# gerbenvoshol/fqzcomp5

Measured on AMD Instinct MI355X. Metric: input MB/s encode+decode, 100MB blocks, -3 and -5; bit-exact vs CPU, higher is better.
Workload: dtype u8

## Files before the change

### fqzcomp5_amd/csrc/block.cpp

```cpp
#include <atomic>
#include <cstdio>
#include <algorithm>
#include <cstdlib>
#include <cstring>
#include <exception>
#include <functional>
#include <thread>
#include <deque>
#include <memory>
#include <vector>

#include "../../include/fqz5_block.h"
#include "rans_codec.hpp"
#include "fqz_codec.hpp"
#include "seq_codec.hpp"
#include "seq_cm.h"
#include "lzp_codec.hpp"
#include "names.hpp"
#include "host_dec.hpp"
#include "rans_format.hpp"

namespace fqz5 {

GpuCtx &gpu();
// ... 22 lines not shown

SeqEncReq seq_req(const fqz5_section &S, int m) {
    static const int slevel[] = {10, 12, 12, 13, 14}, both[] = {0, 0, 1, 1, 1};
    SeqEncReq r;
    r.d_in = S.in;
    r.n = S.in_size;
    r.lens = S.rec_len;
    r.nrec = S.nrec;
    r.k = slevel[m - SEQ10];
    r.both = both[m - SEQ10];
    return r;
}
int seq_strat(int m) {
    static const int slevel[] = {10, 12, 12, 13, 14}, both[] = {0, 0, 1, 1, 1};
    return (slevel[m - SEQ10] << 4) | (both[m - SEQ10] << 3) | 1;
}

int method_order(int m, uint32_t fixed_len) {
    static const int ord[] = {0, 1, 64, 65, 128, 129, 192, 193};
    if (m >= RANS0 && m <= RANS193) return ord[m - RANS0];
    return int((fixed_len << 8) + 9);
}

uint32_t metrics_method(fqz5_trial_state &st, int sec, uint32_t avail) {
    fqz5_section_stats &s = st.sec[sec];
    if (s.review <= 0) {
        s.review = FQZ5_METRICS_REVIEW;
        s.trial = FQZ5_METRICS_TRIAL;
        std::memset(s.usize, 0, sizeof s.usize);
        std::memset(s.csize, 0, sizeof s.csize);
        std::memset(s.count, 0, sizeof s.count);
    }
    if (s.trial > 0) return avail;
    if (s.trial > -99999) {
        int best_m = 0;
        double best = 1e30;
        for (int m = 0; m < FQZ5_M_LAST; m++) {
            if (s.usize[m] && best > (s.csize[m] + 1.0) / s.usize[m]) {
                best = (s.csize[m] + 1.0) / s.usize[m];
                best_m = m;
            }
        }
        s.method_used = best_m;
        s.trial = -99999;
        return 1u << best_m;
    }
    s.review--;
    return 1u << s.method_used;
}

}

struct TrySession {
    std::vector<CompressReq> reqs;
    std::vector<std::vector<int>> req_of;
    std::vector<FqzEncReq> fqz;
    std::vector<uint64_t> fqz_lb;
    std::vector<std::vector<int>> fqz_of;
    std::vector<SeqEncReq> seq;
    std::vector<uint64_t> seq_lb;
    std::vector<uint64_t> fqz_ub, seq_ub;
    std::vector<char> fqz_skip, seq_skip;
    std::vector<std::vector<int>> seq_of;
    std::vector<uint32_t> upper;
    std::deque<std::vector<uint32_t>> recs;
    std::vector<NameEnc> names;
    std::vector<std::vector<int>> name_of;
    bool open = false;
    bool aux = false;
};

FqzEncReq fqz_req(const fqz5_section &S, int m, std::deque<std::vector<uint32_t>> &keep) {
    FqzEncReq r;
    r.d_in = S.in;
    r.n = S.in_size;
    r.nrec = S.nrec;
    keep.emplace_back(S.rec_len, S.rec_len + std::max(S.nrec, 0));
    r.lens = keep.back().data();
    if (S.rec_flags)
        keep.emplace_back(S.rec_flags, S.rec_flags + std::max(S.nrec, 0));
    else
        keep.emplace_back(size_t(std::max(S.nrec, 0)), 0u);
    r.flags = keep.back().data();
    r.d_seq = S.seq;
    r.vers = 4;
    r.strat = m - FQZ0;
    return r;
}
thread_local TrySession t_sess;

void encode_name_jobs(GpuCtx &g, const fqz5_section *secs, const std::vector<int> &which,
                      const std::vector<int> &meth, std::vector<NameEnc> &out) {
// ... 17 lines not shown
        g.download(hb, S.in, S.in_size);
        hipEvent_t e;
        FQZ5_HIP(hipEventCreateWithFlags(&e, hipEventDisableTiming));
        evs.push_back(e);
        FQZ5_HIP(hipEventRecord(e, g.stream));
        host.push_back(hb);
    }
    std::vector<const uint8_t *> h(which.size()), d(which.size());
    std::vector<uint32_t> lens(which.size());
    std::vector<hipEvent_t> ready(which.size());
    for (size_t k = 0; k < which.size(); k++) {
        h[k] = host[size_t(host_of[k])];
        ready[k] = evs[size_t(host_of[k])];
        d[k] = secs[which[k]].in;
        lens[k] = secs[which[k]].in_size;
    }
    names_encode_batch(g, out, h, d, lens, meth, &ready);
    g.sync();
}

std::atomic<int> g_prune{0};
std::atomic<int> g_bounds{0};
std::atomic<uint64_t> g_fqz_tried{0}, g_fqz_pruned{0};
std::atomic<uint64_t> g_chains_host{0}, g_chains_gpu{0};

template <class LB>
std::vector<char> prune_plan(const std::vector<CompressReq> &reqs,
                             const std::vector<std::vector<int>> &of, int mlo, int mhi,
                             size_t nreq, LB lb) {
    std::vector<char> skip(nreq, 0);
    const int nsec = int(of.size());
    std::vector<int> F;
    for (int i = 0; i < nsec; i++)
        for (int m = mlo; m <= mhi; m++)
            if (of[i][m] >= 0) { F.push_back(i); break; }
    if (F.size() != size_t(FQZ5_METRICS_TRIAL)) return skip;
    auto rsize = [&](int i, int m) -> int64_t {
        const int ri = t_sess.req_of[i][m];
        return ri >= 0 && reqs[size_t(ri)].ok ? int64_t(layout_size(reqs[size_t(ri)].out)) : -1;
    };
    std::vector<int64_t> best(F.size(), -1);
    for (size_t k = 0; k < F.size(); k++)
        for (int m = 1; m < mlo; m++) {
            const int64_t z = rsize(F[k], m);
            if (z >= 0 && (best[k] < 0 || z < best[k])) best[k] = z;
        }
// ... 81 lines not shown
    out2[0] = g_chains_host.load();
    out2[1] = g_chains_gpu.load();
}

void fqz5_rans_chain_counts(uint64_t *out2) { rans_chain_counts(out2); }
void fqz5_rans_enc_chain_counts(uint64_t *out2) { rans_enc_chain_counts(out2); }

void fqz5_rans_variant_counts(uint64_t *dec, uint64_t *dec_hedged, uint64_t *enc, int *ndec,
                              int *nenc) {
    rans_variant_counts(dec, dec_hedged, enc, ndec, nenc);
}
const char *fqz5_rans_variant_name(int dir, int i) { return rans_variant_name(dir, i); }

int fqz5_seq_path_counts(uint64_t *out, int n) { return seq_path_counts(out, n); }

void fqz5_trial_counts(uint64_t *out2) {
    out2[0] = g_fqz_tried.load();
    out2[1] = g_fqz_pruned.load();
}

void fqz5_trial_schedule(const int32_t *sec_ids, int nsec, const uint32_t *avail,
                         const fqz5_trial_state *st, uint32_t *masks_out) {
    fqz5_trial_state s = *st;
    for (int i = 0; i < nsec; i++) {
        fqz5_section_stats &ss = s.sec[sec_ids[i]];
        if (ss.review <= 0) {
            ss.review = FQZ5_METRICS_REVIEW;
            ss.trial = FQZ5_METRICS_TRIAL;
        }
        masks_out[i] = 0;
        if (ss.trial > 0) {
            masks_out[i] = avail[sec_ids[i]];
            ss.trial--;
        } else if (ss.trial > -99999) {
            ss.trial = -99999;
        } else {
            ss.review--;
        }
    }
}

using host::now_ms;
using host::now_ns;
using host::step_trace;

int fqz5_sections_try(const fqz5_section *secs, int nsec, const uint32_t *masks,
                      uint32_t *sizes) {
    const double t0 = step_trace() ? now_ms() : 0;
    try {
        GpuCtx &g = gpu();
        if (t_sess.open) {
            g.reset();
            gpu_aux_reset_all();
        }
        t_sess = TrySession();
        for (int i = 0; i < nsec; i++) {
            if (masks[i] & ~(RANS_MASK | FQZ_MASK | SEQ_MASK | NAME_MASK | (1u << LZP3)))
                throw GpuError("fqz5_sections_try: method mask has SEQ_CUSTOM (not in this build)");
            if ((masks[i] & NAME_MASK) && secs[i].sec != FQZ5_SEC_NAME)
                throw GpuError("fqz5_sections_try: name methods need a name section");
            if (secs[i].sec == FQZ5_SEC_NAME && (masks[i] & ~NAME_MASK))
                throw GpuError("fqz5_sections_try: a name section takes name methods only");
            if ((masks[i] & SEQ_MASK) && (secs[i].sec != FQZ5_SEC_SEQ || !secs[i].rec_len))
                throw GpuError("fqz5_sections_try: SEQ methods need a sequence section with records");
            if ((masks[i] & FQZ_MASK) && (secs[i].sec != FQZ5_SEC_QUAL || !secs[i].rec_len))
                throw GpuError("fqz5_sections_try: FQZ methods need a quality section with records");
        }
        std::vector<CompressReq> &reqs = t_sess.reqs;
        t_sess.req_of.assign(nsec, std::vector<int>(FQZ5_M_LAST, -1));
        t_sess.fqz_of.assign(nsec, std::vector<int>(FQZ5_M_LAST, -1));
        t_sess.seq_of.assign(nsec, std::vector<int>(FQZ5_M_LAST, -1));
        t_sess.name_of.assign(nsec, std::vector<int>(FQZ5_M_LAST, -1));
        std::vector<int> name_sec, name_meth;
        std::vector<int> lzp_sec;
        std::vector<CompressReq> sreq;
        std::vector<int> sreq_sec;
        for (int i = 0; i < nsec; i++) {
            const fqz5_section &S = secs[i];
// ... 23 lines not shown
                CompressReq r;
                r.d_in = S.in;
                r.n = S.in_size;
                r.order = method_order(m, S.fixed_len);
                r.cap = compress_bound(r.n, r.order);
                if (m == RANSXN1) {
                    sreq_sec.push_back(i);
                    sreq.push_back(std::move(r));
                    continue;
                }
                t_sess.req_of[i][m] = int(reqs.size());
                reqs.push_back(std::move(r));
            }
        }
        static const bool no_aux = std::getenv("FQZ5_NO_AUX") != nullptr;
        std::vector<FqzEncReq> &fq = t_sess.fqz;
        std::vector<SeqEncReq> &sq = t_sess.seq;
        auto join_stripes = [&] {
            for (size_t k = 0; k < sreq.size(); k++) {
                t_sess.req_of[size_t(sreq_sec[k])][RANSXN1] = int(reqs.size());
                reqs.push_back(std::move(sreq[k]));
            }
            sreq.clear();
        };
        if ((!fq.empty() || !sq.empty() || !lzp_sec.empty() || !sreq.empty() || !name_sec.empty()) &&
            !no_aux) {
            t_sess.aux = true;
            GpuCtx &ga = gpu_aux(0), &gb = gpu_aux(2), &gc = gpu_aux(1);
            size_t nsq = std::min<size_t>(sq.size(), size_t(AUX_NSEQ));
            {
                uint64_t mx = 1;
                for (const SeqEncReq &q : sq) mx = std::max<uint64_t>(mx, q.n);
                size_t fr = 0, tot = 0;
                if (hipMemGetInfo(&fr, &tot) != hipSuccess || !tot) tot = size_t(64) << 30;
                const uint64_t fit = (uint64_t(tot) / 4) / (120 * mx);
                nsq = std::max<size_t>(1, std::min<size_t>(nsq, size_t(fit)));
            }
            std::vector<std::vector<SeqEncReq>> sqg(nsq);
            for (size_t k = 0; k < sq.size(); k++) sqg[k % std::max<size_t>(nsq, 1)].push_back(sq[k]);
            std::vector<CompressReq> lzr;
            std::vector<std::vector<int>> lzr_of(size_t(nsec), std::vector<int>(FQZ5_M_LAST, -1));
            std::vector<std::exception_ptr> err(2 + nsq);
            auto on = [t0](GpuCtx &c, std::exception_ptr &e, auto &&fn) {
                return std::thread([&c, &e, fn, t0] {
                    try {
                        FQZ5_HIP(hipSetDevice(c.device));
// ... 31 lines not shown
            std::vector<CompressReq> plain, rest;
            for (size_t k = 0; k < reqs.size(); k++)
                if ((reqs[k].order & ~1) == 0 && reqs[k].n >= (1u << 20)) plain_at.push_back(k);
            if (plain_at.size() == reqs.size()) plain_at.clear();
            for (size_t k : plain_at) is_plain[k] = 1;
            if (!plain_at.empty())
                for (size_t k = 0; k < reqs.size(); k++)
                    (is_plain[k] ? plain : rest).push_back(std::move(reqs[k]));
            GpuCtx &gp = gpu_aux(AUX_PLAIN);
            gp.prof.on = g.prof.on;
            std::exception_ptr perr;
            std::thread tp = on(gp, perr, [&] { if (!plain.empty()) compress_batch(gp, plain); });
            double tc = 0, tpl = 0;
            try {
                compress_batch(g, plain_at.empty() ? reqs : rest);
                if (!plain_at.empty()) {
                    size_t q = 0;
                    for (size_t k = 0; k < reqs.size(); k++)
                        if (!is_plain[k]) reqs[k] = std::move(rest[q++]);
                }
                tc = step_trace() ? now_ms() : 0;
                tp.join();
                tpl = step_trace() ? now_ms() : 0;
            } catch (...) {
                if (tp.joinable()) tp.join();
                for (auto &t : th) t.join();
                ts.join();
                tn.join();
                throw;
            }
            if (perr) {
                for (auto &t : th) t.join();
                ts.join();
                tn.join();
                std::rethrow_exception(perr);
            }
            for (size_t q = 0; q < plain_at.size(); q++) reqs[plain_at[q]] = std::move(plain[q]);
            g.prof.enc_ms += gp.prof.enc_ms;
            g.prof.enc_launches += gp.prof.enc_launches;
            g.prof.enc_bytes += gp.prof.enc_bytes;
            gp.prof = KernelProfile();
            if (step_trace() && !plain_at.empty())
                std::fprintf(stderr, "sections_try: %zu plain rANS candidates on a helper, "
                             "done %.1f ms after the others\n", plain_at.size(), tpl - tc);
            tc = std::max(tc, tpl);
            for (auto &t : th) t.join();
            ts.join();
            tn.join();
            if (serr) std::rethrow_exception(serr);
            if (nerr) std::rethrow_exception(nerr);
            join_stripes();
            if (step_trace())
                std::fprintf(stderr, "sections_try: rANS candidates %.1f ms, helpers waited "
                             "%.1f ms more\n", tc - t0, now_ms() - tc);
            for (auto &e : err)
                if (e) std::rethrow_exception(e);
            for (size_t k = 0; k < sq.size(); k++)
                sq[k] = std::move(sqg[k % std::max<size_t>(nsq, 1)][k / std::max<size_t>(nsq, 1)]);
            for (int i : lzp_sec) {
                t_sess.req_of[size_t(i)][LZP3] = int(reqs.size());
                reqs.push_back(std::move(lzr[size_t(lzr_of[size_t(i)][LZP3])]));
            }
            std::vector<char> skip_f(fq.size(), 0), skip_s(sq.size(), 0);
            if (g_bounds.load()) {
                for (size_t k = 0; k < fq.size(); k++) skip_f[k] = fqz_size_lower_bound(fq[k]) > 0;
                for (size_t k = 0; k < sq.size(); k++) skip_s[k] = seq_size_upper_bound(sq[k]) > 0;
            } else if (g_prune.load()) {
                skip_f = prune_plan(reqs, t_sess.fqz_of, FQZ0, FQZ4, fq.size(),
                                    [&](size_t k) { return fqz_size_lower_bound(fq[k]); });
                skip_s = prune_plan(reqs, t_sess.seq_of, SEQ10, SEQ14B, sq.size(),
                                    [&](size_t k) { return seq_size_lower_bound(sq[k]); });
            }
            std::exception_ptr ferr;
            std::thread tf = on(ga, ferr, [&] { if (!fq.empty()) fqz_encode_finish(ga, fq, &skip_f); });
// ... 3 lines not shown
            } catch (...) {
                tf.join();
                throw;
            }
            tf.join();
            if (ferr) std::rethrow_exception(ferr);
            t_sess.fqz_skip.insert(t_sess.fqz_skip.end(), skip_f.begin(), skip_f.end());
            t_sess.seq_skip.insert(t_sess.seq_skip.end(), skip_s.begin(), skip_s.end());
            for (size_t k = 0; k < fq.size(); k++) {
                t_sess.fqz_lb.push_back(skip_f[k] ? fqz_size_lower_bound(fq[k]) : 0);
                t_sess.fqz_ub.push_back(skip_f[k] ? fqz_size_upper_bound(fq[k]) : 0);
            }
            for (size_t k = 0; k < sq.size(); k++) {
                t_sess.seq_lb.push_back(skip_s[k] ? seq_size_lower_bound(sq[k]) : 0);
                t_sess.seq_ub.push_back(skip_s[k] ? seq_size_upper_bound(sq[k]) : 0);
            }
            g_fqz_tried += fq.size() + sq.size();
            for (char c : skip_f) g_fqz_pruned += c ? 1 : 0;
            for (char c : skip_s) g_fqz_pruned += c ? 1 : 0;
        } else {
            join_stripes();
            add_lzp3(g, secs, lzp_sec, reqs, t_sess.req_of);
            compress_batch(g, reqs);
            encode_name_jobs(g, secs, name_sec, name_meth, t_sess.names);
            if (!fq.empty()) fqz_encode_batch(g, fq);
            if (!sq.empty()) seq_encode_batch(g, sq);
            t_sess.fqz_lb.assign(fq.size(), 0);
            t_sess.seq_lb.assign(sq.size(), 0);
            t_sess.fqz_ub.assign(fq.size(), 0);
            t_sess.seq_ub.assign(sq.size(), 0);
            t_sess.fqz_skip.assign(fq.size(), 0);
            t_sess.seq_skip.assign(sq.size(), 0);
            g_fqz_tried += fq.size() + sq.size();
        }
        t_sess.open = true;
        if (step_trace())
            std::fprintf(stderr, "sections_try: %.1f ms (device / pinned allocations so far %llu, "
                         "frees %llu)\n", now_ms() - t0,
                         (unsigned long long)ChunkPool::alloc_calls().load(),
                         (unsigned long long)ChunkPool::free_calls().load());
        t_sess.upper.assign(size_t(nsec) * FQZ5_M_LAST, 0);
        for (int i = 0; i < nsec; i++) {
            uint32_t stale = UINT32_MAX;
            for (int m = 0; m < FQZ5_M_LAST; m++) {
                const int ri = t_sess.req_of[i][m], fi = t_sess.fqz_of[i][m];
                const int si = t_sess.seq_of[i][m], ni = t_sess.name_of[i][m];
// ... 12 lines not shown
                }
                if (fi >= 0) {
                    const uint64_t lb = t_sess.fqz_lb[size_t(fi)];
                    sz = t_sess.fqz[size_t(fi)].ok ? layout_size(t_sess.fqz[size_t(fi)].out)
                         : lb ? uint32_t(std::min<uint64_t>(lb, UINT32_MAX - 1)) : 0;
                }
                uint32_t up = sz;
                if (si >= 0 && !t_sess.seq[size_t(si)].ok && t_sess.seq_ub[size_t(si)])
                    up = uint32_t(std::min<uint64_t>(t_sess.seq_ub[size_t(si)], UINT32_MAX - 1));
                if (fi >= 0 && !t_sess.fqz[size_t(fi)].ok && t_sess.fqz_ub[size_t(fi)])
                    up = uint32_t(std::min<uint64_t>(t_sess.fqz_ub[size_t(fi)], UINT32_MAX - 1));
                sizes[size_t(i) * FQZ5_M_LAST + m] = sz;
                t_sess.upper[size_t(i) * FQZ5_M_LAST + m] = up;
            }
        }
        return 0;
    } catch (const std::exception &e) {
        fqz5_set_error(e.what());
        t_sess = TrySession();
        try { gpu().reset(); } catch (...) {}
        try { gpu_aux_reset_all(); } catch (...) {}
        return -1;
    }
}

void fqz5_trial_replay(const int32_t *sec_ids, const uint32_t *in_sizes,
                       const uint32_t *sizes, int nsec, const uint32_t *avail,
                       fqz5_trial_state *st, int32_t *methods_out,
                       uint32_t *tried_out) {
    for (int i = 0; i < nsec; i++) {
        const int sec = sec_ids[i];
        fqz5_section_stats &ss = st->sec[sec];
        const uint32_t methods = metrics_method(*st, sec, avail[sec]);
        const bool in_trial = ss.trial > 0;
        uint32_t best_sz = UINT32_MAX;
        int best_m = 0;
        for (int m = 0; m < FQZ5_M_LAST; m++) {
            if (!(methods & (1u << m))) continue;
            const uint32_t out_len = sizes[size_t(i) * FQZ5_M_LAST + m];
            if (best_sz > out_len) { best_sz = out_len; best_m = m; }
        }
        if (!in_trial && __builtin_popcount(methods) == 1) best_m = __builtin_ctz(methods);
        if (in_trial) {
            for (int m = 0; m < FQZ5_M_LAST; m++) {
                if (!(methods & (1u << m)) || ss.trial <= 0) continue;
                ss.usize[m] += in_sizes[i];
// ... 9 lines not shown

int fqz5_sections_commit(const fqz5_section *secs, int nsec, const int32_t *methods,
                         fqz5_section_result *res) {
    const double t0 = step_trace() ? now_ms() : 0;
    try {
        GpuCtx &g = gpu();
        if (!t_sess.open || int(t_sess.req_of.size()) != nsec)
            throw GpuError("fqz5_sections_commit: no matching fqz5_sections_try");
        std::vector<CompressReq> late;
        std::vector<int> late_of(nsec, -1), late_fqz_of(nsec, -1), late_seq_of(nsec, -1);
        std::vector<FqzEncReq> late_fqz;
        std::vector<SeqEncReq> late_seq;
        std::vector<int> late_lzp;
        std::vector<std::vector<int>> late_lzp_of(nsec, std::vector<int>(FQZ5_M_LAST, -1));
        std::vector<int> late_name_sec, late_name_meth, late_name_of(nsec, -1);
        auto coded_fqz = [&](int i, int m) {
            const int f = t_sess.fqz_of[i][m];
            return f >= 0 && !(size_t(f) < t_sess.fqz_skip.size() && t_sess.fqz_skip[size_t(f)]);
        };
        auto coded_seq = [&](int i, int m) {
            const int q = t_sess.seq_of[i][m];
            return q >= 0 && !(size_t(q) < t_sess.seq_skip.size() && t_sess.seq_skip[size_t(q)]);
        };
        for (int i = 0; i < nsec; i++) {
            const int m = methods[i];
            if (m <= 0 || m >= FQZ5_M_LAST || t_sess.req_of[i][m] >= 0 || coded_fqz(i, m) ||
                coded_seq(i, m) || t_sess.name_of[i][m] >= 0)
                continue;
            if (is_name_method(m) && secs[i].sec == FQZ5_SEC_NAME) {
                late_name_of[i] = int(late_name_sec.size());
                late_name_sec.push_back(i);
                late_name_meth.push_back(m);
                continue;
            }
            if (is_seqcm(m) && secs[i].sec == FQZ5_SEC_SEQ && secs[i].rec_len) {
                late_seq_of[i] = int(late_seq.size());
                late_seq.push_back(seq_req(secs[i], m));
                continue;
            }
            if (is_fqz(m) && secs[i].sec == FQZ5_SEC_QUAL && secs[i].rec_len) {
                late_fqz_of[i] = int(late_fqz.size());
                late_fqz.push_back(fqz_req(secs[i], m, t_sess.recs));
                continue;
            }
            if (m == LZP3 && secs[i].sec == FQZ5_SEC_SEQ) {
                late_lzp.push_back(i);
// ... 115 lines not shown
        std::thread([old = std::make_unique<TrySession>(std::move(t_sess))]() mutable {
            old.reset();
        }).detach();
        t_sess = TrySession();
        if (step_trace())
            std::fprintf(stderr, "sections_commit: late encodes %.1f ms, write %.1f ms, sync "
                         "%.1f ms, release %.1f ms\n", t1 - t0, t2 - t1, t3 - t2, now_ms() - t3);
        return 0;
    } catch (const std::exception &e) {
        fqz5_set_error(e.what());
        t_sess = TrySession();
        try { gpu().reset(); } catch (...) {}
        return -1;
    }
}

int fqz5_encode_sections(const fqz5_section *secs, int nsec, const uint32_t *avail,
                         fqz5_trial_state *st, fqz5_section_result *res) {
    std::vector<uint32_t> sizes(size_t(nsec) * FQZ5_M_LAST), masks(nsec);
    std::vector<int32_t> ids(nsec), meth(nsec);
    std::vector<uint32_t> ins(nsec);
    for (int i = 0; i < nsec; i++) { ids[i] = secs[i].sec; ins[i] = secs[i].in_size; }
    for (int i = 0; i < nsec; i++) masks[i] = avail[secs[i].sec];
    if (fqz5_sections_try(secs, nsec, masks.data(), sizes.data())) return -1;
    fqz5_trial_replay(ids.data(), ins.data(), sizes.data(), nsec, avail, st, meth.data(),
                      nullptr);
    return fqz5_sections_commit(secs, nsec, meth.data(), res);
}

int fqz5_decode_sections(const fqz5_section *secs, int nsec, fqz5_section_result *res) {
    struct ExitTrace {
        double t;
        ~ExitTrace() {
            if (t) std::fprintf(stderr, "decode_sections: entry to exit %.1f ms\n", now_ms() - t);
        }
    } exit_trace{step_trace() ? now_ms() : 0.0};
    try {
        GpuCtx &g = gpu();
        const bool trace = step_trace();
        const double t0 = now_ms();
        size_t tot = 0;
        for (int i = 0; i < nsec; i++) tot += secs[i].in_size;
        uint8_t *host = g.staging.alloc(tot + 1);
        size_t off = 0;
        for (int i = 0; i < nsec; i++) {
            g.download(host + off, secs[i].in, secs[i].in_size);
            off += secs[i].in_size;
// ... 395 lines not shown
```

### fqzcomp5_amd/sections.py

```python
from __future__ import annotations

import ctypes as C

import numpy as np

from . import lib as _lib

M_LAST = 31
SEC_NAME, SEC_SEQ, SEC_QUAL = 0, 2, 3
RANS0, RANS1, RANS64, RANS65, RANS128, RANS129, RANS192, RANS193, RANSXN1 = range(1, 10)
LZP3 = 10
TLZP3 = 11
TOK3_3, TOK3_5, TOK3_7, TOK3_9 = range(12, 16)
TOK3_3_LZP, TOK3_5_LZP, TOK3_7_LZP, TOK3_9_LZP = range(16, 20)
NAME_MASK = sum(1 << m for m in range(TLZP3, TOK3_9_LZP + 1))
SEQ10, SEQ12, SEQ12B, SEQ13B, SEQ14B = range(20, 25)
FQZ0, FQZ1, FQZ2, FQZ3, FQZ4 = range(26, 31)
RANS_MASK = sum(1 << m for m in range(RANS0, RANSXN1 + 1))
FQZ_MASK = sum(1 << m for m in range(FQZ0, FQZ4 + 1))
SEQ_MASK = sum(1 << m for m in range(SEQ10, SEQ14B + 1))
WORK_MASK = FQZ_MASK | SEQ_MASK | (1 << LZP3)

PRESET_MASKS = {
    1: {SEC_NAME: [TLZP3],
# ... 69 lines not shown


def _load():
    global _bound
    so = _lib.load()
    if not _bound:
        so.fqz5_trial_init.argtypes = [C.POINTER(TrialState)]
        so.fqz5_set_trial_prune.restype = C.c_int
        so.fqz5_set_trial_prune.argtypes = [C.c_int]
        so.fqz5_set_trial_bounds.restype = C.c_int
        so.fqz5_set_trial_bounds.argtypes = [C.c_int]
        so.fqz5_arenas_release.restype = C.c_int
        so.fqz5_arenas_release.argtypes = []
        so.fqz5_sections_try_upper.restype = C.c_int
        so.fqz5_sections_try_upper.argtypes = [C.POINTER(C.c_uint32), C.c_int]
        so.fqz5_trial_counts.argtypes = [C.POINTER(C.c_uint64)]
        so.fqz5_trial_schedule.argtypes = [C.POINTER(C.c_int32), C.c_int,
                                           C.POINTER(C.c_uint32), C.POINTER(TrialState),
                                           C.POINTER(C.c_uint32)]
        so.fqz5_sections_try.argtypes = [C.POINTER(Section), C.c_int,
                                         C.POINTER(C.c_uint32),
                                         C.POINTER(C.c_uint32)]
        so.fqz5_sections_try.restype = C.c_int
        so.fqz5_trial_replay.argtypes = [C.POINTER(C.c_int32), C.POINTER(C.c_uint32),
                                         C.POINTER(C.c_uint32), C.c_int,
                                         C.POINTER(C.c_uint32), C.POINTER(TrialState),
                                         C.POINTER(C.c_int32), C.POINTER(C.c_uint32)]
        so.fqz5_sections_commit.argtypes = [C.POINTER(Section), C.c_int,
                                            C.POINTER(C.c_int32),
                                            C.POINTER(SectionResult)]
        so.fqz5_sections_commit.restype = C.c_int
        so.fqz5_decode_sections.argtypes = [C.POINTER(Section), C.c_int,
                                            C.POINTER(SectionResult)]
        so.fqz5_decode_sections.restype = C.c_int
        _bound = True
    return so


def masks(level: int, seq_cm: bool = False, full: bool = False) -> np.ndarray:
    av = np.zeros(4, np.uint32)
    for sec, ms in PRESET_MASKS[level].items():
        for m in ms:
            if m not in BUILT or (m in SEQ_PARAMS and not (seq_cm or full)):
                continue
            av[sec] |= np.uint32(1 << m)
    return av


def new_state() -> TrialState:
    st = TrialState()
    _load().fqz5_trial_init(C.byref(st))
    return st


def _arr(t, xs):
    return (t * len(xs))(*xs)


def trial_schedule(sec_ids, avail: np.ndarray, state: TrialState) -> np.ndarray:
    so = _load()
    ids = np.ascontiguousarray(sec_ids, np.int32)
    av = np.ascontiguousarray(avail, np.uint32)
    out = np.zeros(len(ids), np.uint32)
    so.fqz5_trial_schedule(ids.ctypes.data_as(C.POINTER(C.c_int32)), len(ids),
                           av.ctypes.data_as(C.POINTER(C.c_uint32)), C.byref(state),
                           out.ctypes.data_as(C.POINTER(C.c_uint32)))
    return out


def sections_try(secs: list[Section], masks: np.ndarray) -> np.ndarray:
    so = _load()
    sizes = np.zeros(len(secs) * M_LAST, np.uint32)
    av = np.ascontiguousarray(masks, np.uint32)
    assert len(av) == len(secs)
    _lib.after_torch()
    rc = so.fqz5_sections_try(_arr(Section, secs), len(secs),
                              av.ctypes.data_as(C.POINTER(C.c_uint32)),
                              sizes.ctypes.data_as(C.POINTER(C.c_uint32)))
    if rc:
        raise _lib.NativeError("fqz5_sections_try: " + _lib.last_error())
    return sizes.reshape(len(secs), M_LAST)


def trial_replay(sec_ids, in_sizes, sizes: np.ndarray, avail: np.ndarray,
                 state: TrialState, tried: np.ndarray | None = None) -> np.ndarray:
    so = _load()
    n = len(sec_ids)
    ids = np.ascontiguousarray(sec_ids, np.int32)
    ins = np.ascontiguousarray(in_sizes, np.uint32)
    sz = np.ascontiguousarray(sizes, np.uint32).reshape(-1)
    av = np.ascontiguousarray(avail, np.uint32)
    out = np.zeros(n, np.int32)
    so.fqz5_trial_replay(ids.ctypes.data_as(C.POINTER(C.c_int32)),
                         ins.ctypes.data_as(C.POINTER(C.c_uint32)),
                         sz.ctypes.data_as(C.POINTER(C.c_uint32)), n,
                         av.ctypes.data_as(C.POINTER(C.c_uint32)),
                         C.byref(state), out.ctypes.data_as(C.POINTER(C.c_int32)),
                         None if tried is None else
                         tried.ctypes.data_as(C.POINTER(C.c_uint32)))
    return out


def sections_try_bounds(secs: list[Section], masks: np.ndarray):
    so = _load()
    prev = so.fqz5_set_trial_bounds(1)
    try:
        lo = sections_try(secs, masks)
    finally:
        so.fqz5_set_trial_bounds(prev)
    hi = np.zeros(len(secs) * M_LAST, np.uint32)
    if so.fqz5_sections_try_upper(hi.ctypes.data_as(C.POINTER(C.c_uint32)), len(secs)):
        raise _lib.NativeError("fqz5_sections_try_upper: " + _lib.last_error())
    return lo, hi.reshape(len(secs), M_LAST)


def _first_min_open(lo, hi, ratios: bool = False) -> list:
    w = min(range(len(lo)), key=lambda j: (lo[j], j))
    out = []
    for j in range(len(lo)):
        if j == w or (lo[j] == hi[j] and lo[w] == hi[w]):
            continue
        gap = hi[w] * (1 + 1e-9) if ratios else hi[w]
        if (j < w and not gap < lo[j]) or (j > w and not gap <= lo[j]):
            out.append(j)
    return out + [w] if out else []


def _first_min_fixed(lo, hi, ratios: bool = False) -> bool:
    return not _first_min_open(lo, hi, ratios)

# ... 192 lines not shown
    if group is None:
        group = dist.group.WORLD
    ws, rk = _world(group)
    if ws == 1:
        return local, in_sizes, sec_ids, 0
    pack = np.zeros((local.shape[0], M_LAST + 2), np.int64)
    pack[:, :M_LAST] = local
    pack[:, M_LAST] = in_sizes
    pack[:, M_LAST + 1] = sec_ids
    rows = xchg(pack, group)
    allp = np.concatenate(rows, 0)
    off = sum(int(r.shape[0]) for r in rows[:rk])
    return (allp[:, :M_LAST].astype(np.uint32), allp[:, M_LAST].astype(np.uint32),
            allp[:, M_LAST + 1].astype(np.int32), off)


def encode_run(secs: list[Section], avail: np.ndarray, state: TrialState,
               group=None, speculate: bool = True, prune: bool = True,
               bounds: bool = False):
    ins = np.array([s.in_size for s in secs], np.uint32)
    ids = np.array([s.sec for s in secs], np.int32)
    av = np.asarray(avail, np.uint32)
    SPEC = RANS_MASK | NAME_MASK
    if speculate and not (av & WORK_MASK).any():
        masks = av[ids]
        prune = False
    else:
        blank = np.zeros((len(secs), M_LAST), np.uint32)
        _, _, g_ids0, off = exchange_sizes(blank, ins, ids, group)
        sched_all = trial_schedule(g_ids0, avail, state)
        sched = sched_all[off:off + len(secs)]
        NAME_WORK = 1 << TLZP3
        masks = ((av[ids] & np.uint32(SPEC & ~NAME_WORK & 0xFFFFFFFF)) |
                 (sched & np.uint32(WORK_MASK | NAME_WORK)) if speculate else sched)
        for fam in (FQZ_MASK, SEQ_MASK):
            rows = np.nonzero(sched_all & fam)[0]
            if len(rows) == 0:
                continue
            prune = prune and speculate and len(rows) == TRIAL_WINDOW and \
                bool(((rows >= off) & (rows < off + len(secs))).all())
        if bounds and _world(group)[0] == 1 and (sched_all & WORK_MASK).any() and \
                bounds_usable(g_ids0, sched_all, state, final=True):
            global last_bounds_decided
            state0 = _copy_state(state)
            lo, hi = sections_try_bounds(secs, masks)
            tried = np.zeros(len(secs), np.uint32)
            meth_all = trial_replay(ids, ins, lo, avail, state, tried)
            last_bounds_decided = trial_decided(lo, hi, ids, ins, tried, sched_all, state0,
                                                final=True)
            if last_bounds_decided:
                return sections_commit(secs, meth_all), meth_all, lo, tried, 0
            C.memmove(C.byref(state), C.byref(state0), C.sizeof(TrialState))
    so = _load()
    prev = so.fqz5_set_trial_prune(1 if prune else 0)
    try:
        local = sections_try(secs, masks)
    finally:
        so.fqz5_set_trial_prune(prev)
    g_sizes, g_ins, g_ids, off = exchange_sizes(local, ins, ids, group)
    tried = np.zeros(len(g_ids), np.uint32)
    meth_all = trial_replay(g_ids, g_ins, g_sizes, avail, state, tried)
    meth = meth_all[off:off + len(secs)]
    res = sections_commit(secs, meth)
    return res, meth_all, g_sizes, tried, off


def _chunks(rows, sizes, budget: int):
    out, cur, tot = [], [], 0
    for i in rows:
        if cur and tot + int(sizes[i]) > budget:
            out.append(cur)
            cur, tot = [], 0
        cur.append(i)
        tot += int(sizes[i])
    if cur:
        out.append(cur)
    return out


# ... 58 lines not shown
            tried = np.zeros(len(g_ids), np.uint32)
            meth_all = trial_replay(g_ids, g_ins, g_sizes, avail, state, tried)
        global last_bounds_decided
        last_bounds_decided = ok
        if not ok:
            print(f"[sections] size intervals do not decide the trial ({why[0] if why else ''}): "
                  "trying again with exact sizes", file=sys.stderr, flush=True)
            C.memmove(C.byref(state), C.byref(state0), C.sizeof(TrialState))
            lo, _ = try_all(False)
            g_sizes, g_ins, g_ids, off = exchange_sizes(lo, ins, ids, group)
            tried = np.zeros(len(g_ids), np.uint32)
            meth_all = trial_replay(g_ids, g_ins, g_sizes, avail, state, tried)
    meth = meth_all[off:off + len(secs)]
    if bounds and last_bounds_decided and session:
        return sections_commit(secs, meth), meth_all, g_sizes, tried, off
    if so.fqz5_arenas_release():
        raise _lib.NativeError("fqz5_arenas_release: " + _lib.last_error())
    res = []
    for ch in _chunks(range(len(secs)), ins, max(commit_bytes, chunk_bytes)):
        part = [secs[i] for i in ch]
        sections_try(part, np.zeros(len(ch), np.uint32))
        res += sections_commit(part, meth[ch])
    return res, meth_all, g_sizes, tried, off


def _world(group):
    import torch.distributed as dist
    if group is None or not dist.is_available() or not dist.is_initialized():
        return 1, 0
    return dist.get_world_size(group), dist.get_rank(group)


def allreduce_min(a: np.ndarray, group) -> np.ndarray:
    if _world(group)[0] == 1:
        return a
    parts = xchg(np.ascontiguousarray(a, np.int64), group)
    return np.minimum.reduce(parts).astype(a.dtype)


def work_share(methods: list[int], world: int, rank: int) -> int:
    m = 0
    for j, meth in enumerate(sorted(methods)):
        if j % world == rank:
            m |= 1 << meth
    return m

# ... 454 lines not shown
```

### include/fqz5_block.h

```cpp
#ifndef FQZ5_BLOCK_H
#define FQZ5_BLOCK_H
#include <stdint.h>

#ifdef __cplusplus
extern "C" {
#endif

#define FQZ5_M_LAST 31
#define FQZ5_SEC_NAME 0
#define FQZ5_SEC_LEN 1
#define FQZ5_SEC_SEQ 2
#define FQZ5_SEC_QUAL 3
#define FQZ5_SEC_LAST 4
#define FQZ5_METRICS_REVIEW 100
#define FQZ5_METRICS_TRIAL 3

typedef struct {
    uint64_t usize[FQZ5_M_LAST], csize[FQZ5_M_LAST];
    int32_t review, trial;
    int32_t count[FQZ5_M_LAST];
    int32_t method_used;
} fqz5_section_stats;

typedef struct {
// ... 17 lines not shown
    int32_t method;
    int32_t strat;
    int32_t status;
    uint32_t clen;
    uint32_t usize;
} fqz5_section_result;

void fqz5_trial_init(fqz5_trial_state *st);

int fqz5_encode_sections(const fqz5_section *secs, int n, const uint32_t *avail,
                         fqz5_trial_state *st, fqz5_section_result *res);

void fqz5_trial_schedule(const int32_t *sec_ids, int n, const uint32_t *avail,
                         const fqz5_trial_state *st, uint32_t *masks_out);
int fqz5_sections_try(const fqz5_section *secs, int n, const uint32_t *masks,
                      uint32_t *sizes);
void fqz5_trial_replay(const int32_t *sec_ids, const uint32_t *in_sizes,
                       const uint32_t *sizes, int n, const uint32_t *avail,
                       fqz5_trial_state *st, int32_t *methods_out,
                       uint32_t *tried_out );
int fqz5_sections_commit(const fqz5_section *secs, int n, const int32_t *methods,
                         fqz5_section_result *res);

int fqz5_set_trial_prune(int on);
int fqz5_set_trial_bounds(int on);
int fqz5_sections_try_upper(uint32_t *upper, int nsec);
int fqz5_arenas_release(void);
void fqz5_trial_counts(uint64_t *out2);

int fqz5_decode_sections(const fqz5_section *secs, int n, fqz5_section_result *res);


#define FQZ5_FREAD2 128

void fqz5_name_flags(const char *names, uint32_t name_len, int nrec, uint32_t *flags);

int fqz5_block_lengths(const uint32_t *len, int nrec, int32_t fixed_len, uint8_t *out,
                       uint32_t cap);

typedef struct {
    int32_t nrec;
    const uint8_t *name;
    uint32_t name_size;
    const uint8_t *lengths;
    uint32_t lengths_size;
    const uint8_t *seq;
// ... 38 lines not shown
```

Before: 3562.

## Stage trial encoding so follower sections only encode the predicted winner

Adds a staged trial path. Sections still inside the trial window are encoded with every candidate method. Sections whose method is already settled are restricted to that method, and sections that follow a trial window get no encodes in the first pass. After the trial-window encodes finish, the best rANS method is picked from the accumulated stats and only that method is encoded for the followers, split across a helper context. This cuts redundant candidate encodes per batch, at the cost of a second encode stage and possible mispredictions that must be fixed up in replay.

Result: faster. 4326, median of 6 (+21.5%).

```diff
diff --git a/fqzcomp5_amd/csrc/block.cpp b/fqzcomp5_amd/csrc/block.cpp
--- a/fqzcomp5_amd/csrc/block.cpp
+++ b/fqzcomp5_amd/csrc/block.cpp
@@ -68,6 +68,19 @@
     return int((fixed_len << 8) + 9);
 }
 
+int pick_method(const fqz5_section_stats &s, uint32_t among) {
+    int best_m = 0;
+    double best = 1e30;
+    for (int m = 0; m < FQZ5_M_LAST; m++) {
+        if (!(among & (1u << m))) continue;
+        if (s.usize[m] && best > (s.csize[m] + 1.0) / s.usize[m]) {
+            best = (s.csize[m] + 1.0) / s.usize[m];
+            best_m = m;
+        }
+    }
+    return best_m;
+}
+
 uint32_t metrics_method(fqz5_trial_state &st, int sec, uint32_t avail) {
     fqz5_section_stats &s = st.sec[sec];
     if (s.review <= 0) {
@@ -79,20 +92,98 @@
     }
     if (s.trial > 0) return avail;
     if (s.trial > -99999) {
-        int best_m = 0;
-        double best = 1e30;
-        for (int m = 0; m < FQZ5_M_LAST; m++) {
-            if (s.usize[m] && best > (s.csize[m] + 1.0) / s.usize[m]) {
-                best = (s.csize[m] + 1.0) / s.usize[m];
-                best_m = m;
-            }
-        }
-        s.method_used = best_m;
+        s.method_used = pick_method(s, ~0u);
         s.trial = -99999;
-        return 1u << best_m;
+        return 1u << s.method_used;
     }
     s.review--;
     return 1u << s.method_used;
+}
+
+enum TrialStep { STEP_TRIAL, STEP_DECIDE, STEP_KEEP };
+TrialStep trial_step(fqz5_section_stats &ss, bool *fresh = nullptr) {
+    if (ss.review <= 0) {
+        ss.review = FQZ5_METRICS_REVIEW;
+        ss.trial = FQZ5_METRICS_TRIAL;
+        if (fresh) *fresh = true;
+    }
+    if (ss.trial > 0) {
+        ss.trial--;
+        return STEP_TRIAL;
+    }
+    if (ss.trial > -99999) {
+        ss.trial = -99999;
+        return STEP_DECIDE;
+    }
+    ss.review--;
+    return STEP_KEEP;
+}
+
+struct Decision {
+    int kind = 0;
+    bool fresh = false;
+    std::vector<int> rows;
+    std::vector<int> follow;
+};
+
+void staged_walk(const int32_t *sec_ids, int nsec, const uint32_t *avail,
+                 const fqz5_trial_state *st, int32_t *roles, uint32_t *masks, int32_t *window,
+                 std::vector<Decision> *decs) {
+    fqz5_trial_state s = *st;
+    int cur[FQZ5_SEC_LAST], nwin[FQZ5_SEC_LAST], settled[FQZ5_SEC_LAST];
+    bool open[FQZ5_SEC_LAST];
+    for (int k = 0; k < FQZ5_SEC_LAST; k++) {
+        cur[k] = -1;
+        nwin[k] = 0;
+        settled[k] = s.sec[k].method_used;
+        open[k] = false;
+    }
+    std::vector<Decision> local;
+    std::vector<Decision> &D = decs ? *decs : local;
+    for (int i = 0; i < nsec; i++) {
+        const int k = sec_ids[i];
+        fqz5_section_stats &ss = s.sec[k];
+        const bool staged = k == FQZ5_SEC_SEQ || k == FQZ5_SEC_QUAL;
+        bool fresh = false;
+        const TrialStep step = trial_step(ss, &fresh);
+        window[i] = -1;
+        if (step == STEP_TRIAL) {
+            roles[i] = staged ? FQZ5_ROLE_TRIAL : FQZ5_ROLE_OTHER;
+            masks[i] = avail[k];
+            if (!staged) continue;
+            if (!open[k]) {
+                Decision d;
+                d.kind = k;
+                d.fresh = fresh;
+                cur[k] = int(D.size());
+                D.push_back(d);
+                open[k] = true;
+                nwin[k]++;
+            }
+            D[size_t(cur[k])].rows.push_back(i);
+            window[i] = nwin[k] - 1;
+            continue;
+        }
+        if (!staged) {
+            roles[i] = FQZ5_ROLE_OTHER;
+            masks[i] = 0;
+            continue;
+        }
+        if (step == STEP_DECIDE && !open[k]) {
+            settled[k] = pick_method(st->sec[k], ~0u);
+            cur[k] = -1;
+        }
+        open[k] = false;
+        if (cur[k] >= 0) {
+            roles[i] = FQZ5_ROLE_FOLLOW;
+            masks[i] = 0;
+            window[i] = nwin[k] - 1;
+            D[size_t(cur[k])].follow.push_back(i);
+        } else {
+            roles[i] = FQZ5_ROLE_SETTLED;
+            masks[i] = 1u << settled[k];
+        }
+    }
 }
 
 }
@@ -114,6 +205,7 @@
     std::vector<std::vector<int>> name_of;
     bool open = false;
     bool aux = false;
+    std::vector<int> predicted;
 };
 
 FqzEncReq fqz_req(const fqz5_section &S, int m, std::deque<std::vector<uint32_t>> &keep) {
@@ -177,6 +269,19 @@
 std::atomic<int> g_prune{0};
 std::atomic<int> g_bounds{0};
 std::atomic<uint64_t> g_fqz_tried{0}, g_fqz_pruned{0};
+std::atomic<int> g_staged{-1};
+std::atomic<uint64_t> g_staged_n[4];
+std::atomic<uint64_t> g_staged_dec[FQZ5_SEC_LAST];
+bool staged_on() {
+    int v = g_staged.load();
+    if (v < 0) {
+        const char *e = std::getenv("FQZ5_STAGED_TRY");
+        v = !(e && e[0] == '0');
+        int want = -1;
+        if (!g_staged.compare_exchange_strong(want, v)) v = want;
+    }
+    return v != 0;
+}
 std::atomic<uint64_t> g_chains_host{0}, g_chains_gpu{0};
 
 template <class LB>
@@ -304,30 +409,39 @@
 void fqz5_trial_schedule(const int32_t *sec_ids, int nsec, const uint32_t *avail,
                          const fqz5_trial_state *st, uint32_t *masks_out) {
     fqz5_trial_state s = *st;
-    for (int i = 0; i < nsec; i++) {
-        fqz5_section_stats &ss = s.sec[sec_ids[i]];
-        if (ss.review <= 0) {
-            ss.review = FQZ5_METRICS_REVIEW;
-            ss.trial = FQZ5_METRICS_TRIAL;
-        }
-        masks_out[i] = 0;
-        if (ss.trial > 0) {
-            masks_out[i] = avail[sec_ids[i]];
-            ss.trial--;
-        } else if (ss.trial > -99999) {
-            ss.trial = -99999;
-        } else {
-            ss.review--;
-        }
-    }
+    for (int i = 0; i < nsec; i++)
+        masks_out[i] = trial_step(s.sec[sec_ids[i]]) == STEP_TRIAL ? avail[sec_ids[i]] : 0;
+}
+
+void fqz5_staged_plan(const int32_t *sec_ids, int nsec, const uint32_t *avail,
+                      const fqz5_trial_state *st, int32_t *roles_out, uint32_t *masks_out,
+                      int32_t *window_out) {
+    staged_walk(sec_ids, nsec, avail, st, roles_out, masks_out, window_out, nullptr);
+}
+
+int fqz5_set_staged_try(int on) {
+    const int prev = staged_on();
+    g_staged.store(on ? 1 : 0);
+    return prev;
+}
+
+void fqz5_staged_counts(uint64_t out[4]) {
+    for (int k = 0; k < 4; k++) out[k] = g_staged_n[k].load();
+}
+
+void fqz5_staged_decisions(uint64_t out[FQZ5_SEC_LAST]) {
+    for (int k = 0; k < FQZ5_SEC_LAST; k++) out[k] = g_staged_dec[k].load();
 }
 
 using host::now_ms;
 using host::now_ns;
 using host::step_trace;
 
-int fqz5_sections_try(const fqz5_section *secs, int nsec, const uint32_t *masks,
-                      uint32_t *sizes) {
+}
+
+static int sections_try_impl(const fqz5_section *secs, int nsec, const uint32_t *masks_in,
+                             uint32_t *sizes, const uint32_t *avail,
+                             const fqz5_trial_state *st) {
     const double t0 = step_trace() ? now_ms() : 0;
     try {
         GpuCtx &g = gpu();
@@ -336,6 +450,26 @@
             gpu_aux_reset_all();
         }
         t_sess = TrySession();
+        t_sess.predicted.assign(size_t(std::max(nsec, 0)), -1);
+        std::vector<uint32_t> stage1(masks_in, masks_in + std::max(nsec, 0));
+        std::vector<Decision> decs;
+        const bool staged = avail && st && staged_on() && nsec > 0;
+        if (staged) {
+            std::vector<int32_t> ids(nsec), roles(nsec), win(nsec);
+            std::vector<uint32_t> pm(nsec);
+            for (int i = 0; i < nsec; i++) ids[i] = secs[i].sec;
+            staged_walk(ids.data(), nsec, avail, st, roles.data(), pm.data(), win.data(), &decs);
+            uint64_t skipped = 0;
+            for (int i = 0; i < nsec; i++) {
+                if (roles[i] == FQZ5_ROLE_SETTLED) stage1[i] &= pm[i];
+                if (roles[i] == FQZ5_ROLE_FOLLOW) stage1[i] = 0;
+                uint32_t gone = masks_in[i] & ~stage1[i];
+                if (!secs[i].fixed_len) gone &= ~(1u << RANSXN1);
+                skipped += uint64_t(__builtin_popcount(gone));
+            }
+            g_staged_n[3] += skipped;
+        }
+        const uint32_t *masks = stage1.data();
         for (int i = 0; i < nsec; i++) {
             if (masks[i] & ~(RANS_MASK | FQZ_MASK | SEQ_MASK | NAME_MASK | (1u << LZP3)))
                 throw GpuError("fqz5_sections_try: method mask has SEQ_CUSTOM (not in this build)");
@@ -405,6 +539,89 @@
                 reqs.push_back(std::move(sreq[k]));
             }
             sreq.clear();
+        };
+        if (staged)
+            g_staged_n[0] += reqs.size() + sreq.size() + lzp_sec.size() + fq.size() + sq.size();
+        auto stage2 = [&](GpuCtx *plain_ctx) {
+            std::vector<CompressReq> s2;
+            std::vector<int> s2_sec, s2_m;
+            for (const Decision &d : decs) {
+                fqz5_section_stats s = st->sec[d.kind];
+                if (d.fresh) {
+                    std::memset(s.usize, 0, sizeof s.usize);
+                    std::memset(s.csize, 0, sizeof s.csize);
+                }
+                if (d.follow.empty()) continue;
+                for (int i : d.rows)
+                    for (int m = 1; m < FQZ5_M_LAST; m++) {
+                        if (!(masks_in[i] & RANS_MASK & (1u << m))) continue;
+                        const int ri = t_sess.req_of[size_t(i)][m];
+                        s.usize[m] += secs[i].in_size;
+                        s.csize[m] += ri < 0 ? UINT32_MAX
+                                      : reqs[size_t(ri)].ok ? layout_size(reqs[size_t(ri)].out) : 0;
+                    }
+                const int w = pick_method(s, RANS_MASK);
+                g_staged_dec[d.kind]++;
+                if (step_trace())
+                    std::fprintf(stderr, "sections_try: staged: kind %d decided at %.1f ms: method %d "
+                                 "for %zu sections\n", d.kind, now_ms() - t0, w, d.follow.size());
+                if (!w) continue;
+                for (int i : d.follow) {
+                    const fqz5_section &S = secs[i];
+                    if (!(masks_in[i] & (1u << w)) || (w == RANSXN1 && !S.fixed_len)) continue;
+                    CompressReq r;
+                    r.d_in = S.in;
+                    r.n = S.in_size;
+                    r.order = method_order(w, S.fixed_len);
+                    r.cap = compress_bound(r.n, r.order);
+                    s2.push_back(std::move(r));
+                    s2_sec.push_back(i);
+                    s2_m.push_back(w);
+                }
+            }
+            if (s2.empty()) return;
+            std::vector<CompressReq> pl, rest;
+            std::vector<char> is_pl(s2.size(), 0);
+            for (size_t k = 0; k < s2.size(); k++)
+                is_pl[k] = plain_ctx && (s2[k].order & ~1) == 0 && s2[k].n >= (1u << 20);
+            for (size_t k = 0; k < s2.size(); k++) (is_pl[k] ? pl : rest).push_back(std::move(s2[k]));
+            if (pl.empty() || rest.empty()) {
+                compress_batch(g, pl.empty() ? rest : pl);
+            } else {
+                std::exception_ptr e2;
+                plain_ctx->prof.on = g.prof.on;
+                std::thread t2([&] {
+                    try {
+                        FQZ5_HIP(hipSetDevice(plain_ctx->device));
+                        compress_batch(*plain_ctx, pl);
+                    } catch (...) {
+                        e2 = std::current_exception();
+                    }
+                });
+                try {
+                    compress_batch(g, rest);
+                } catch (...) {
+                    t2.join();
+                    throw;
+                }
+                t2.join();
+                if (e2) std::rethrow_exception(e2);
+                g.prof.enc_ms += plain_ctx->prof.enc_ms;
+                g.prof.enc_launches += plain_ctx->prof.enc_launches;
+                g.prof.enc_bytes += plain_ctx->prof.enc_bytes;
+                plain_ctx->prof = KernelProfile();
+            }
+            size_t qp = 0, qr = 0;
+            for (size_t k = 0; k < s2_sec.size(); k++) {
+                t_sess.req_of[size_t(s2_sec[k])][s2_m[k]] = int(reqs.size());
+                t_sess.predicted[size_t(s2_sec[k])] = s2_m[k];
+                reqs.push_back(std::move(is_pl[k] ? pl[qp++] : rest[qr++]));
+            }
+            g_staged_n[1] += s2_sec.size();
+            g_staged_n[3] -= s2_sec.size();
+            if (step_trace())
+                std::fprintf(stderr, "sections_try: staged: stage 2 (%zu sections) done at %.1f ms\n",
+                             s2_sec.size(), now_ms() - t0);
         };
         if ((!fq.empty() || !sq.empty() || !lzp_sec.empty() || !sreq.empty() || !name_sec.empty()) &&
             !no_aux) {
@@ -482,34 +699,30 @@
                 tc = step_trace() ? now_ms() : 0;
                 tp.join();
                 tpl = step_trace() ? now_ms() : 0;
+                ts.join();
+                if (perr) std::rethrow_exception(perr);
+                if (serr) std::rethrow_exception(serr);
+                for (size_t q = 0; q < plain_at.size(); q++) reqs[plain_at[q]] = std::move(plain[q]);
+                g.prof.enc_ms += gp.prof.enc_ms;
+                g.prof.enc_launches += gp.prof.enc_launches;
+                g.prof.enc_bytes += gp.prof.enc_bytes;
+                gp.prof = KernelProfile();
+                if (step_trace() && !plain_at.empty())
+                    std::fprintf(stderr, "sections_try: %zu plain rANS candidates on a helper, "
+                                 "done %.1f ms after the others\n", plain_at.size(), tpl - tc);
+                join_stripes();
+                if (staged) stage2(&gp);
+                tc = step_trace() ? now_ms() : 0;
             } catch (...) {
                 if (tp.joinable()) tp.join();
+                if (ts.joinable()) ts.join();
                 for (auto &t : th) t.join();
-                ts.join();
                 tn.join();
                 throw;
             }
-            if (perr) {
-                for (auto &t : th) t.join();
-                ts.join();
-                tn.join();
-                std::rethrow_exception(perr);
-            }
-            for (size_t q = 0; q < plain_at.size(); q++) reqs[plain_at[q]] = std::move(plain[q]);
-            g.prof.enc_ms += gp.prof.enc_ms;
-            g.prof.enc_launches += gp.prof.enc_launches;
-            g.prof.enc_bytes += gp.prof.enc_bytes;
-            gp.prof = KernelProfile();
-            if (step_trace() && !plain_at.empty())
-                std::fprintf(stderr, "sections_try: %zu plain rANS candidates on a helper, "
-                             "done %.1f ms after the others\n", plain_at.size(), tpl - tc);
-            tc = std::max(tc, tpl);
             for (auto &t : th) t.join();
-            ts.join();
             tn.join();
-            if (serr) std::rethrow_exception(serr);
             if (nerr) std::rethrow_exception(nerr);
-            join_stripes();
             if (step_trace())
                 std::fprintf(stderr, "sections_try: rANS candidates %.1f ms, helpers waited "
                              "%.1f ms more\n", tc - t0, now_ms() - tc);
@@ -559,6 +772,7 @@
             join_stripes();
             add_lzp3(g, secs, lzp_sec, reqs, t_sess.req_of);
             compress_batch(g, reqs);
+            if (staged) stage2(nullptr);
             encode_name_jobs(g, secs, name_sec, name_meth, t_sess.names);
             if (!fq.empty()) fqz_encode_batch(g, fq);
             if (!sq.empty()) seq_encode_batch(g, sq);
@@ -617,6 +831,19 @@
         try { gpu_aux_reset_all(); } catch (...) {}
         return -1;
     }
+}
+
+extern "C" {
+
+int fqz5_sections_try(const fqz5_section *secs, int nsec, const uint32_t *masks,
+                      uint32_t *sizes) {
+    return sections_try_impl(secs, nsec, masks, sizes, nullptr, nullptr);
+}
+
+int fqz5_sections_try_staged(const fqz5_section *secs, int nsec, const uint32_t *masks,
+                             uint32_t *sizes, const uint32_t *avail,
+                             const fqz5_trial_state *st) {
+    return sections_try_impl(secs, nsec, masks, sizes, avail, st);
 }
 
 void fqz5_trial_replay(const int32_t *sec_ids, const uint32_t *in_sizes,
@@ -672,6 +899,10 @@
             const int q = t_sess.seq_of[i][m];
             return q >= 0 && !(size_t(q) < t_sess.seq_skip.size() && t_sess.seq_skip[size_t(q)]);
         };
+        for (int i = 0; i < nsec; i++)
+            if (size_t(i) < t_sess.predicted.size() && t_sess.predicted[size_t(i)] >= 0 &&
+                t_sess.predicted[size_t(i)] != methods[i])
+                g_staged_n[2]++;
         for (int i = 0; i < nsec; i++) {
             const int m = methods[i];
             if (m <= 0 || m >= FQZ5_M_LAST || t_sess.req_of[i][m] >= 0 || coded_fqz(i, m) ||
@@ -833,7 +1064,7 @@
     std::vector<uint32_t> ins(nsec);
     for (int i = 0; i < nsec; i++) { ids[i] = secs[i].sec; ins[i] = secs[i].in_size; }
     for (int i = 0; i < nsec; i++) masks[i] = avail[secs[i].sec];
-    if (fqz5_sections_try(secs, nsec, masks.data(), sizes.data())) return -1;
+    if (fqz5_sections_try_staged(secs, nsec, masks.data(), sizes.data(), avail, st)) return -1;
     fqz5_trial_replay(ids.data(), ins.data(), sizes.data(), nsec, avail, st, meth.data(),
                       nullptr);
     return fqz5_sections_commit(secs, nsec, meth.data(), res);
diff --git a/fqzcomp5_amd/sections.py b/fqzcomp5_amd/sections.py
--- a/fqzcomp5_amd/sections.py
+++ b/fqzcomp5_amd/sections.py
@@ -115,6 +115,18 @@
                                          C.POINTER(C.c_uint32),
                                          C.POINTER(C.c_uint32)]
         so.fqz5_sections_try.restype = C.c_int
+        if hasattr(so, "fqz5_sections_try_staged"):
+            so.fqz5_sections_try_staged.argtypes = [C.POINTER(Section), C.c_int,
+                                                    C.POINTER(C.c_uint32), C.POINTER(C.c_uint32),
+                                                    C.POINTER(C.c_uint32), C.POINTER(TrialState)]
+            so.fqz5_sections_try_staged.restype = C.c_int
+            so.fqz5_staged_plan.argtypes = [C.POINTER(C.c_int32), C.c_int, C.POINTER(C.c_uint32),
+                                            C.POINTER(TrialState), C.POINTER(C.c_int32),
+                                            C.POINTER(C.c_uint32), C.POINTER(C.c_int32)]
+            so.fqz5_set_staged_try.restype = C.c_int
+            so.fqz5_set_staged_try.argtypes = [C.c_int]
+            so.fqz5_staged_counts.argtypes = [C.POINTER(C.c_uint64)]
+            so.fqz5_staged_decisions.argtypes = [C.POINTER(C.c_uint64)]
         so.fqz5_trial_replay.argtypes = [C.POINTER(C.c_int32), C.POINTER(C.c_uint32),
                                          C.POINTER(C.c_uint32), C.c_int,
                                          C.POINTER(C.c_uint32), C.POINTER(TrialState),
@@ -161,15 +173,58 @@
     return out
 
 
-def sections_try(secs: list[Section], masks: np.ndarray) -> np.ndarray:
+ROLE_TRIAL, ROLE_SETTLED, ROLE_FOLLOW, ROLE_OTHER = range(4)
+
+
+def staged_plan(sec_ids, avail: np.ndarray, state: TrialState):
+    so = _load()
+    ids = np.ascontiguousarray(sec_ids, np.int32)
+    av = np.ascontiguousarray(avail, np.uint32)
+    roles = np.zeros(len(ids), np.int32)
+    out = np.zeros(len(ids), np.uint32)
+    win = np.zeros(len(ids), np.int32)
+    so.fqz5_staged_plan(ids.ctypes.data_as(C.POINTER(C.c_int32)), len(ids),
+                        av.ctypes.data_as(C.POINTER(C.c_uint32)), C.byref(state),
+                        roles.ctypes.data_as(C.POINTER(C.c_int32)),
+                        out.ctypes.data_as(C.POINTER(C.c_uint32)),
+                        win.ctypes.data_as(C.POINTER(C.c_int32)))
+    return roles, out, win
+
+
+def set_staged_try(on: bool) -> bool:
+    return bool(_load().fqz5_set_staged_try(1 if on else 0))
+
+
+def staged_counts() -> tuple[int, int, int, int]:
+    out = (C.c_uint64 * 4)()
+    _load().fqz5_staged_counts(out)
+    return tuple(int(x) for x in out)
+
+
+def staged_decisions() -> list[int]:
+    out = (C.c_uint64 * 4)()
+    _load().fqz5_staged_decisions(out)
+    return [int(x) for x in out]
+
+
+def sections_try(secs: list[Section], masks: np.ndarray, state: TrialState | None = None,
+                 avail: np.ndarray | None = None) -> np.ndarray:
     so = _load()
     sizes = np.zeros(len(secs) * M_LAST, np.uint32)
     av = np.ascontiguousarray(masks, np.uint32)
     assert len(av) == len(secs)
     _lib.after_torch()
-    rc = so.fqz5_sections_try(_arr(Section, secs), len(secs),
-                              av.ctypes.data_as(C.POINTER(C.c_uint32)),
-                              sizes.ctypes.data_as(C.POINTER(C.c_uint32)))
+    if state is not None:
+        avl = np.ascontiguousarray(avail, np.uint32)
+        rc = so.fqz5_sections_try_staged(_arr(Section, secs), len(secs),
+                                         av.ctypes.data_as(C.POINTER(C.c_uint32)),
+                                         sizes.ctypes.data_as(C.POINTER(C.c_uint32)),
+                                         avl.ctypes.data_as(C.POINTER(C.c_uint32)),
+                                         C.byref(state))
+    else:
+        rc = so.fqz5_sections_try(_arr(Section, secs), len(secs),
+                                  av.ctypes.data_as(C.POINTER(C.c_uint32)),
+                                  sizes.ctypes.data_as(C.POINTER(C.c_uint32)))
     if rc:
         raise _lib.NativeError("fqz5_sections_try: " + _lib.last_error())
     return sizes.reshape(len(secs), M_LAST)
@@ -194,11 +249,12 @@
     return out
 
 
-def sections_try_bounds(secs: list[Section], masks: np.ndarray):
+def sections_try_bounds(secs: list[Section], masks: np.ndarray, state: TrialState | None = None,
+                        avail: np.ndarray | None = None):
     so = _load()
     prev = so.fqz5_set_trial_bounds(1)
     try:
-        lo = sections_try(secs, masks)
+        lo = sections_try(secs, masks, state, avail)
     finally:
         so.fqz5_set_trial_bounds(prev)
     hi = np.zeros(len(secs) * M_LAST, np.uint32)
@@ -437,6 +493,9 @@
     ids = np.array([s.sec for s in secs], np.int32)
     av = np.asarray(avail, np.uint32)
     SPEC = RANS_MASK | NAME_MASK
+    staged = state if speculate and _one_rank(group) and \
+        hasattr(_load(), "fqz5_sections_try_staged") and \
+        bounds_usable(ids, (), state, final=True) else None
     if speculate and not (av & WORK_MASK).any():
         masks = av[ids]
         prune = False
@@ -458,7 +517,7 @@
                 bounds_usable(g_ids0, sched_all, state, final=True):
             global last_bounds_decided
             state0 = _copy_state(state)
-            lo, hi = sections_try_bounds(secs, masks)
+            lo, hi = sections_try_bounds(secs, masks, staged, av)
             tried = np.zeros(len(secs), np.uint32)
             meth_all = trial_replay(ids, ins, lo, avail, state, tried)
             last_bounds_decided = trial_decided(lo, hi, ids, ins, tried, sched_all, state0,
@@ -469,7 +528,7 @@
     so = _load()
     prev = so.fqz5_set_trial_prune(1 if prune else 0)
     try:
-        local = sections_try(secs, masks)
+        local = sections_try(secs, masks, staged, av)
     finally:
         so.fqz5_set_trial_prune(prev)
     g_sizes, g_ins, g_ids, off = exchange_sizes(local, ins, ids, group)
@@ -574,6 +633,13 @@
         sections_try(part, np.zeros(len(ch), np.uint32))
         res += sections_commit(part, meth[ch])
     return res, meth_all, g_sizes, tried, off
+
+
+def _one_rank(group) -> bool:
+    import torch.distributed as dist
+    if not dist.is_available() or not dist.is_initialized():
+        return True
+    return dist.get_world_size(dist.group.WORLD if group is None else group) == 1
 
 
 def _world(group):
diff --git a/include/fqz5_block.h b/include/fqz5_block.h
--- a/include/fqz5_block.h
+++ b/include/fqz5_block.h
@@ -63,6 +63,20 @@
 int fqz5_sections_commit(const fqz5_section *secs, int n, const int32_t *methods,
                          fqz5_section_result *res);
 
+#define FQZ5_ROLE_TRIAL 0
+#define FQZ5_ROLE_SETTLED 1
+#define FQZ5_ROLE_FOLLOW 2
+#define FQZ5_ROLE_OTHER 3
+int fqz5_sections_try_staged(const fqz5_section *secs, int n, const uint32_t *masks,
+                             uint32_t *sizes, const uint32_t *avail,
+                             const fqz5_trial_state *st);
+void fqz5_staged_plan(const int32_t *sec_ids, int n, const uint32_t *avail,
+                      const fqz5_trial_state *st, int32_t *roles_out, uint32_t *masks_out,
+                      int32_t *window_out);
+int fqz5_set_staged_try(int on);
+void fqz5_staged_counts(uint64_t out[4]);
+void fqz5_staged_decisions(uint64_t out[FQZ5_SEC_LAST]);
+
 int fqz5_set_trial_prune(int on);
 int fqz5_set_trial_bounds(int on);
 int fqz5_sections_try_upper(uint32_t *upper, int nsec);
```
